# skim0119/gym-softrobot

Measured on AMD Instinct MI355X. Metric: env_steps_per_sec, higher is better.
Workload: dtype f64

## Files before the change

### gym_softrobot_amd/csrc/softrod_capi.hip

```cpp
#include <hip/hip_runtime.h>
#include <hip/hip_ext.h>

#include <cmath>
#include <cstdio>
#include <cstdlib>
#include <cstring>
#include <new>
#include <string>
#include <vector>

#include "softrod_kernels.hpp"
#include "softrod_dynamics_readout.hpp"
#include "softrod_copy_envs.hpp"
#include "softrod_state_bank.hpp"
#include "softrod_episode_stats.hpp"
#include "softrod_shape.hpp"
#include "softrod_reset_shapes.hpp"

using namespace softrod;

template <class Row>
struct EnvTable {
    Row* dev = nullptr;
    Row* host = nullptr;
// ... 39 lines not shown
    bool window_paired = true;
    std::string tier;
    RodParams P{};
    StatePtrs S{};
    std::vector<void*> owned;
    double* d_init = nullptr;
    uint8_t* d_mask = nullptr;
    double* d_basis = nullptr;
    double* d_spline = nullptr;
    bool spline_set = false;
    RodParams* d_params = nullptr;
    StatePtrs* d_state = nullptr;
    double* d_time_tab = nullptr;
    double* d_mat = nullptr;
    double* d_render_radius = nullptr;
    double* d_mtab = nullptr;
    bool muscles_set = false;
    unsigned* d_ticket = nullptr;
    bool tapered = false;
    bool was_reset = false;
    bool basis_set = false;
    double* h_init = nullptr;
    uint8_t* h_mask = nullptr;
    std::vector<hipEvent_t> ev_start, ev_stop;
    int timed = 0;
    hipEvent_t ev_reset = nullptr;
    int q_depth = 0;
    double* d_queue = nullptr;
    double* h_queue = nullptr;
    int* d_consumed = nullptr;
    int* d_produced = nullptr;
    int* d_underflow = nullptr;
    uint8_t* d_flags = nullptr;
    int* h_produced = nullptr;
    std::vector<int> seen_consumed;
    std::vector<int2> pending;
    double* h_stage = nullptr;
    int2* h_where = nullptr;
    double* d_stage = nullptr;
    int2* d_where = nullptr;
    size_t stage_cap = 0;
    int* h_status = nullptr;
    hipEvent_t ev_status = nullptr;
    bool status_pending = false;
    hipEvent_t ev_queue = nullptr;
    bool same_step = false;
// ... 275 lines not shown
    }
    SR_HIP(h, hipGetLastError());
    return SOFTROD_OK;
}

enum : unsigned { kOptMuscles = SOFTROD_FEAT_COOMM_MUSCLES, kOptEarlyTerm = kFeatEarlyTerm, kOptEnvMaterial = kFeatEnvMaterial,
                  kOptEnvContact = kFeatEnvContact, kOptCompiledFor = kOptEarlyTerm | kOptEnvMaterial | kOptEnvContact };
constexpr int kAny = -1, kMoctoEnvs = -2;
constexpr unsigned kAnyFeatures = kRuntimeFeatures;
using StepKernel = void (*)(RodParams, StatePtrs, const float*, float*, double*, uint8_t*, uint8_t*, double*, int, int, int);
using OctoKernel = void (*)(RodParams, StatePtrs, const float*, float*, double*, uint8_t*, uint8_t*, int, int, int);
using WindowKernel = void (*)(RodParams, StatePtrs, const float*, int, int);

struct StepRow {
    unsigned feats;
    int env;
    int math, epl;
    int taper, zup;
    int nw_min, nw_max;
    bool windowed;
    unsigned needs, honours;
    StepKernel step; OctoKernel octo; WindowKernel window;
    bool cert;
    int epb, waves;
    const char* label;
};

constexpr StepRow compiled_row(unsigned F, int env, int epl, int taper, int nw_min, int nw_max, const char* label) {
    const bool rt = F == kRuntimeFeatures;
    StepRow r{};
    r.feats = rt ? kAnyFeatures : F & ~(kFeatPlaneZup | kOptCompiledFor);
    r.env = env; r.math = SOFTROD_MATH_FAST; r.epl = epl; r.taper = taper; r.nw_min = nw_min; r.nw_max = nw_max;
    r.zup = rt ? kAny : (F & kFeatPlaneZup) != 0;
    r.needs = rt ? 0u : F & kOptCompiledFor;
    r.honours = rt ? 0u : F & (kOptCompiledFor | kOptMuscles);
    r.epb = 1; r.label = label;
    return r;
}
template <unsigned F, int E, int EPL, bool TAPER = false>
constexpr StepRow fast_row(const char* label) {
    StepRow r = compiled_row(F, E, EPL, TAPER, 1, 1, label);
    r.step = softrod_step_fast_kernel<F, E, EPL, TAPER>;
    r.cert = (F & ~kFeatEnvMaterial) == SOFTROD_FEATURES_SOFTPENDULUM;
    return r;
}
template <unsigned F, int MAXW, int EPB>
constexpr StepRow octo_row(int env, int nw_min, int nw_max, const char* label) {
    StepRow r = compiled_row(F, env, 1, kAny, nw_min, nw_max, label);
    r.octo = softrod_octo_step_kernel<F, MAXW, EPB>;
    r.epb = EPB; r.waves = EPB == 1 ? 0 : MAXW * EPB;
    return r;
}
template <unsigned F, int RPB>
constexpr StepRow window_row(const char* label) {
    StepRow r = compiled_row(F, SOFTROD_ENV_ARM_SINGLE, 2, 0, 1, 1, label);
    r.window = softrod_step_window_kernel<F, RPB>;
    r.windowed = true; r.epb = RPB; r.waves = 2 * RPB;
    return r;
}
template <bool ET>
constexpr StepRow libm_row(unsigned feats, int env, int zup, int taper, unsigned honours) {
    StepRow r{};
    r.feats = feats; r.env = env; r.math = SOFTROD_MATH_LIBM; r.epl = 1; r.taper = taper; r.zup = zup;
    r.nw_min = r.nw_max = r.epb = 1;
    r.needs = ET ? kOptEarlyTerm : 0u; r.honours = r.needs | kOptMuscles | honours;
    r.step = softrod_step_libm_kernel<ET>;
// ... 144 lines not shown
        SR_HIP(h, hipMalloc((void**)&T.dev, N * sizeof(Row)));
        SR_HIP(h, hipHostMalloc((void**)&T.host, N * sizeof(Row), hipHostMallocDefault));
        SR_HIP(h, hipEventCreateWithFlags(&T.ev, hipEventDisableTiming));
        Row R0;
        build(own, R0);
        for (size_t i = 0; i < N; ++i) T.host[i] = R0;
        if (const hipError_t e = bank_adopt_table(h, T.dev, R0)) {
            T.release();
            T = EnvTable<Row>{};
            return fail(h, SOFTROD_EHIP, std::string("state bank: ") + hipGetErrorString(e));
        }
        slot = T.dev;
        SR_HIP(h, hipMemcpy(h->d_state, &h->S, sizeof(StatePtrs), hipMemcpyHostToDevice));
    } else {
        SR_HIP(h, hipEventSynchronize(T.ev));
    }
    for (size_t i = 0; i < N; ++i)
        if (!mask || mask[i]) build(values + W * i, T.host[i]);
    SR_HIP(h, hipMemcpyAsync(T.dev, T.host, N * sizeof(Row), hipMemcpyHostToDevice, st));
    SR_HIP(h, hipEventRecord(T.ev, st));
    return SOFTROD_OK;
}

template <class K, class... A>
void launch_stamped(K kernel, const dim3& grid, const dim3& block, hipStream_t st, hipEvent_t t0, hipEvent_t t1, A... args) {
    if (t0 || t1) hipExtLaunchKernelGGL(kernel, grid, block, 0, st, t0, t1, 0, args...);
    else hipLaunchKernelGGL(kernel, grid, block, 0, st, args...);
}

int launch_step(softrod_handle* h, const float* actions, float* obs, double* reward,
                uint8_t* term, uint8_t* trunc, double* aux, int n_sub, int epilogue, int pack,
                hipStream_t st) {
    if (h->q_depth > 0 && epilogue && !h->same_step) {
        if (const int rc = launch_autoreset(h, obs, reward, term, trunc, aux, pack, st)) return rc;
        if (h->rs_count > 0)
            if (const int rc = launch_reset_shapes(h, kPickSkipped, nullptr, obs, term, trunc, aux, pack, st)) return rc;
    }
    if ((h->cfg.features & SOFTROD_FEAT_COOMM_MUSCLES) && h->cfg.math_mode == SOFTROD_MATH_FAST) {
        const bool push = h->cfg.env_kind == SOFTROD_ENV_ARM_PUSH || is_pull(h) || is_mocto(h);
        if (is_mocto(h) && (!h->tapered || !h->muscles_set || (h->cfg.env_kind == SOFTROD_ENV_ARM_TWO && !h->basis_set)))
            return fail(h, SOFTROD_EINVAL, "the muscle octopus needs softrod_set_radius_profile and softrod_set_muscle_layers "
                                           "(and SOFTROD_ENV_ARM_TWO softrod_set_action_basis) before it steps");
        if (push && !h->tapered)
            return fail(h, SOFTROD_EINVAL, "SOFTROD_ENV_ARM_PUSH (SOFTROD_MATH_FAST): call softrod_set_radius_profile first "
                                           "(the reference's arm is tapered, arm_push_env.py:160-179)");
        if (!push && h->tapered)
            return fail(h, SOFTROD_EINVAL, "a tapered muscle rod outside SOFTROD_ENV_ARM_PUSH runs under SOFTROD_MATH_LIBM only");
    }
    const StepChoice c = select_step(h, epilogue);
    if (!c.row) return fail(h, SOFTROD_EINVAL, c.why);
    const StepChoice after = c.row->windowed ? select_step(h, 0) : StepChoice{nullptr, nullptr};
    if (c.row->windowed && !after.row) return fail(h, SOFTROD_EINVAL, after.why);
    if (c.row->cert) h->cert_live = true;
    else if (const int rc = clear_planar_certs(h, st, false)) return rc;
    auto launch = [&](const StepRow& r, int n, int epi, hipEvent_t t0, hipEvent_t t1) {
        const dim3 grid((unsigned)((h->cfg.n_envs + r.epb - 1) / r.epb)), block(kLanes * (r.waves ? r.waves : h->nw));
        if (r.window) launch_stamped(r.window, grid, block, st, t0, t1, h->P, h->S, actions, n, h->window_refresh);
        else if (r.octo) launch_stamped(r.octo, grid, block, st, t0, t1, h->P, h->S, actions, obs, reward, term, trunc, n, epi, pack);
        else launch_stamped(r.step, grid, block, st, t0, t1, h->P, h->S, actions, obs, reward, term, trunc, aux, n, epi, pack);
    };
    const bool timing = h->timed < (int)h->ev_start.size();
    const hipEvent_t t0 = timing ? h->ev_start[h->timed] : nullptr, t1 = timing ? h->ev_stop[h->timed] : nullptr;
    const bool mocto = c.row->env == kMoctoEnvs;
    const bool action_first = mocto && epilogue && actions, epilogue_last = mocto && epilogue;
    const dim3 grid((unsigned)h->cfg.n_envs), block(kLanes * h->nw);
    if (action_first)
        launch_stamped(softrod_mocto_action_kernel, grid, block, st, t0, nullptr, h->P, h->S, actions, n_sub);
    launch(*c.row, n_sub, epilogue, action_first ? nullptr : t0, (after.row || epilogue_last) ? nullptr : t1);
    if (after.row) launch(*after.row, 0, 1, nullptr, epilogue_last ? nullptr : t1);
    if (epilogue_last)
        launch_stamped(softrod_mocto_epilogue_kernel, grid, block, st, nullptr, t1, h->P, h->S, obs, reward, term, trunc, 1, pack);
    SR_HIP(h, hipGetLastError());
    if (timing) ++h->timed;
    if (h->q_depth > 0 && epilogue && h->same_step) {
        if (const int rc = launch_autoreset_same_step(h, obs, aux, pack, st)) return rc;
        if (h->rs_count > 0)
            if (const int rc = launch_reset_shapes(h, kPickFinished, nullptr, obs, term, trunc, aux, pack, st)) return rc;
    }
    return SOFTROD_OK;
}

int upload_and_reset(softrod_handle* h, hipStream_t st, bool use_mask) {
    const size_t N = (size_t)h->cfg.n_envs;
    if (const int rc = clear_planar_certs(h, st)) return rc;
    SR_HIP(h, hipMemcpyAsync(h->d_init, h->h_init, N * h->init_stride * sizeof(double), hipMemcpyHostToDevice, st));
    if (use_mask)
        SR_HIP(h, hipMemcpyAsync(h->d_mask, h->h_mask, N, hipMemcpyHostToDevice, st));
    ResetArgs A{h->d_init, use_mask ? h->d_mask : nullptr};
    if (is_octo(h)) {
        OctoResetArgs OA{h->d_init, h->d_init + N * (size_t)h->cfg.n_arm * 18, use_mask ? h->d_mask : nullptr};
        hipLaunchKernelGGL(softrod_octo_reset_kernel, dim3((unsigned)N), dim3(kLanes * h->nw), 0, st, h->P, h->S, OA);
    } else
        hipLaunchKernelGGL(by_epl(h, softrod_reset_kernel<1>, softrod_reset_kernel<2>), dim3((unsigned)N), dim3(kLanes), 0, st,
                           h->P, h->S, A);
// ... 1848 lines not shown
    if (!h->S.planar_cert) return SOFTROD_OK;
    SR_ON_DEVICE(h);
    SR_HIP(h, hipDeviceSynchronize());
    std::vector<uint8_t> bytes((size_t)h->cfg.n_envs + 1, 0);
    bytes.back() = on ? 1 : 0;
    SR_HIP(h, hipMemcpy(h->S.planar_cert, bytes.data(), bytes.size(), hipMemcpyHostToDevice));
    h->cert_live = false;
    h->cert_on = on != 0;
    return SOFTROD_OK;
}

int softrod_planar_certificates(softrod_handle* h, uint8_t* out, void* stream) {
    if (!h || !out) return fail(h, SOFTROD_EINVAL, "planar certificates: null argument");
    SR_ON_DEVICE(h);
    const size_t N = (size_t)h->cfg.n_envs;
    if (!h->S.planar_cert) SR_HIP(h, hipMemsetAsync(out, 0, N, (hipStream_t)stream));
    else SR_HIP(h, hipMemcpyAsync(out, h->S.planar_cert, N, hipMemcpyDeviceToDevice, (hipStream_t)stream));
    return SOFTROD_OK;
}

int softrod_set_timing(softrod_handle* h, int n_launches) {
    if (!h || n_launches < 0 || n_launches > (1 << 20)) return fail(h, SOFTROD_EINVAL, "bad argument");
    SR_ON_DEVICE(h);
    while ((int)h->ev_start.size() < n_launches) {
        hipEvent_t a = nullptr, b = nullptr;
        SR_HIP(h, hipEventCreate(&a));
        SR_HIP(h, hipEventCreate(&b));
        h->ev_start.push_back(a);
        h->ev_stop.push_back(b);
    }
    while ((int)h->ev_start.size() > n_launches) {
        (void)hipEventDestroy(h->ev_start.back());
        (void)hipEventDestroy(h->ev_stop.back());
        h->ev_start.pop_back();
        h->ev_stop.pop_back();
    }
    h->timed = 0;
    return SOFTROD_OK;
}

int softrod_kernel_times_ms(softrod_handle* h, float* out_ms, int cap, int* count) {
    if (!h || !out_ms || !count || cap < 0) return fail(h, SOFTROD_EINVAL, "bad argument");
    SR_ON_DEVICE(h);
    const int n = h->timed < cap ? h->timed : cap;
    for (int i = 0; i < n; ++i) {
        SR_HIP(h, hipEventSynchronize(h->ev_stop[i]));
        SR_HIP(h, hipEventElapsedTime(out_ms + i, h->ev_start[i], h->ev_stop[i]));
    }
    *count = n;
    return SOFTROD_OK;
}

int softrod_last_kernel_ms(softrod_handle* h, float* ms) {
    if (!h || !ms) return fail(h, SOFTROD_EINVAL, "null argument");
    if (h->timed < 1) return fail(h, SOFTROD_EINVAL, "timing not enabled or no timed launch yet");
    SR_ON_DEVICE(h);
    SR_HIP(h, hipEventSynchronize(h->ev_stop[h->timed - 1]));
    SR_HIP(h, hipEventElapsedTime(ms, h->ev_start[h->timed - 1], h->ev_stop[h->timed - 1]));
    return SOFTROD_OK;
}

const char* softrod_last_error(softrod_handle* h) { return h ? h->err.c_str() : g_err.c_str(); }

const char* softrod_kernel_tier(softrod_handle* h) {
    if (!h) return "";
    const StepChoice c = select_step(h);
    std::string t = c.row ? c.row->label : std::string("none: ") + c.why;
    auto fill = [&t](const char* token, const std::string& with) {
        const size_t at = t.find(token);
        if (at != std::string::npos) t.replace(at, std::strlen(token), with);
    };
    fill("{waves}", std::to_string(h->nw) + (h->nw == 1 ? " wave" : " waves"));
    fill("{refresh}", std::to_string(h->window_refresh));
    if (c.row && c.row->windowed)
        if (const StepRow* after = select_step(h, 0).row) t += std::string(" + ") + after->label + " epilogue";
    if (h->env_mat.dev) t += ",env material";
    if (h->env_contact.dev) t += ",env contact";
    h->tier = t;
    return h->tier.c_str();
}

int softrod_destroy(softrod_handle* h) {
    if (!h) return SOFTROD_OK;
    DeviceGuard guard_(h->device);
    (void)hipDeviceSynchronize();
    autoreset_release(h);
    for (void* p : h->owned) (void)hipFree(p);
    for (double* p : h->d_rs_field) if (p) (void)hipFree(p);
    if (h->h_init) (void)hipHostFree(h->h_init);
    h->env_mat.release();
    h->env_contact.release();
    if (h->h_mask) (void)hipHostFree(h->h_mask);
    for (hipEvent_t e : h->ev_start) (void)hipEventDestroy(e);
    for (hipEvent_t e : h->ev_stop) (void)hipEventDestroy(e);
    if (h->ev_reset) (void)hipEventDestroy(h->ev_reset);
    if (h->h_pairs) (void)hipHostFree(h->h_pairs);
    if (h->ev_pairs) (void)hipEventDestroy(h->ev_pairs);
    h->bank.release();
    if (h->d_stats) (void)hipFree(h->d_stats);
    delete h;
    return SOFTROD_OK;
}

}

#ifdef SOFTROD_PHASE_CLOCKS
extern "C" int softrod_debug_phase_clocks(unsigned long long* out, int n_rods) {
    return (int)hipMemcpyFromSymbol(out, HIP_SYMBOL(softrod::g_phase_clock), (size_t)n_rods * 8 * sizeof(unsigned long long));
}
#endif
```

### gym_softrobot_amd/csrc/softrod_fast.hpp

```cpp
#pragma once

namespace softrod {

__device__ __forceinline__ bool wave_any(bool p) { return __builtin_amdgcn_ballot_w64(p) != 0ull; }
__device__ __forceinline__ bool wave_any_of(unsigned long long lanes, bool p) {
    return (__builtin_amdgcn_ballot_w64(p) & lanes) != 0ull;
}

__device__ __forceinline__ double horner(double g, double y, double c) {
    double d;
    asm("v_fma_f64 %0, %1, %2, %3" : "=v"(d) : "v"(g), "v"(y), "v"(c));
    return d;
}
__device__ __forceinline__ void fma_over(double& d, double a, double b, double c) {
    asm("v_fma_f64 %0, %1, %2, %3" : "+v"(d) : "v"(a), "v"(b), "v"(c));
}
__device__ __forceinline__ void fma_inplace_u(double& x, double m, double a) {
    asm("v_fma_f64 %0, %1, %0, %2" : "+v"(x) : "s"(m), "v"(a));
}

template <bool LEAN = true, bool ON_CIRCLE = false>
__device__ __forceinline__ void sinc_cosc(double t, double& sc, double& cc) {
    if (!wave_any(t >= 1.0e-3)) {
        if constexpr (LEAN) {
// ... 542 lines not shown
constexpr int fast_kernel_waves() {
    if (EPL > 1) return 1;
    if (F == kRuntimeFeatures) return SOFTROD_RUNTIME_WAVES;
    if (F & (SOFTROD_FEAT_PLANE_CONTACT_ANISO | SOFTROD_FEAT_LAPLACE_FILTER | SOFTROD_FEAT_SPLINE_MUSCLE_TORQUES |
             SOFTROD_FEAT_COOMM_MUSCLES))
        return SOFTROD_CONTACT_WAVES;
    if (TAPER) return SOFTROD_CONTACT_WAVES;
    return (F & ~kFeatEnvMaterial) == SOFTROD_FEATURES_SOFTPENDULUM ? SOFTROD_PLANAR_WAVES : SOFTROD_FAST_WAVES;
}

template <unsigned F, int E, int EPL, bool TAPER = false>
__global__ void __launch_bounds__(kLanes, (fast_kernel_waves<F, EPL, TAPER>()))
softrod_step_fast_kernel(const RodParams P, const StatePtrs S, const float* __restrict__ actions,
                         float* __restrict__ obs, double* __restrict__ reward,
                         uint8_t* __restrict__ terminated, uint8_t* __restrict__ truncated,
                         double* __restrict__ aux, const int n_sub, const int epilogue, const int pack) {
    const int rod = blockIdx.x;
    const int lane = threadIdx.x;
    const size_t N = (size_t)P.n_envs;
    [[maybe_unused]] EnvMaterial M;
    if constexpr (kEnvMaterial<F>) M = S.env_mat[rod];
    [[maybe_unused]] EnvContact CT;
    if constexpr (kEnvContact<F>) CT = S.env_contact[rod];
    if (epilogue && S.skip && S.skip[rod]) {
        if (lane == 0) S.skip[rod] = 0;
        if (lane == 0 && early_term_on<F>(P)) S.aux[rod] = 0.0;
        return;
    }

    __builtin_amdgcn_s_setprio(3);
    SR_PHASE(0);
    constexpr bool kPlanarKernel = (F & ~kFeatEnvMaterial) == SOFTROD_FEATURES_SOFTPENDULUM;
    LaneN<EPL> L;
    BcTargets B;
    EnvAction A;
    [[maybe_unused]] bool certified = false, cert_on = false, proof_ok = true, proof_nan = false;
    [[maybe_unused]] double s2w = 1.0;
    bool blown_up = false;
    if constexpr (kPlanarKernel) {
        unsigned cert = 0, on = 0;
        if (S.planar_cert) { on = S.planar_cert[N]; cert = S.planar_cert[rod]; }
        double bc_in_plane[3];
        planar_load_state<EPL>(S, N, rod, lane, L, bc_in_plane);
        set_action_n<F, E, EPL>(P, S, N, rod, lane, actions, A, B, L);
        cert_on = __builtin_amdgcn_readfirstlane((int)on) != 0;
        cert = cert_on ? (unsigned)__builtin_amdgcn_readfirstlane((int)cert) : 0u;
// ... 24 lines not shown
    if constexpr (kEnvMaterial<F>) build_const_m<F, EPL, TAPER>(P, M, lane, A, C, S.mat);
    else build_const_m<F, EPL, TAPER>(P, P, lane, A, C, S.mat);
    if constexpr (kEnvContact<F>) C.ct = CT;
    if constexpr (kMusclesCompiled<F>) build_muscle_const<F, EPL, true>(P, S, N, rod, lane, A, C);
    RodParams Pk = P;
    if (!has<F>(P, SOFTROD_FEAT_ANALYTICAL_DAMPER)) Pk.damp_t = 1.0;

    if constexpr (kPlanarKernel) {
        blown_up = n_sub > 0 && epilogue && __any(proof_nan || planar_has_nan<EPL>(P, lane, L));
    } else if (n_sub > 0 && epilogue && rod_has_nan<EPL>(P, lane, L)) {
        blown_up = true;
        poison_rod<EPL>(L);
        time = clock_after(P, S, time, n_sub);
    }
    if constexpr (kPlanarKernel) {
        PlanarN<EPL> Z;
        const bool planar = n_sub > 0 && !blown_up && !__any(!(planar_from_lane<EPL>(P, lane, L, s2w, Z) && proof_ok));
        if (__builtin_expect(planar, 1)) {
            PlanarC<EPL> K;
            planar_build_const<EPL, kEnvMaterial<F>>(Pk, C, lane, K);
            const double ta = P.time_two_half_adds ? P.half_dt : P.dt;
            const double tb = P.time_two_half_adds ? P.half_dt : 0.0;
            int tk = -1;
            if (S.time_tab && n_sub == P.tab_n_sub) {
                const double kf = rint(time * P.inv_step_time);
                const int k = (kf >= 0.0 && kf < (double)(P.tab_len - 1)) ? (int)kf : -1;
                tk = (k >= 0 && S.time_tab[k] == time) ? k : -1;
            }
            const double step_dt = EPL > 1 ? opaque_v(P.dt) : P.dt;
            SR_PHASE(2);
#if SOFTROD_PLANAR_EXEC_MASK
            if (lane * EPL <= P.n_elem) {
#endif
                planar_kinematic_n<EPL>(P.half_dt, K.hq_hdt, C, K, Z);
                {
                    int s = 0;
#pragma unroll
                    for (int q = 0; q < 4; ++q) {
                        if (q == 1) __builtin_amdgcn_s_setprio(2);
                        if (q == 2) __builtin_amdgcn_s_setprio(1);
                        if (q == 3) __builtin_amdgcn_s_setprio(0);
                        const int end = ProgressPriority::bound(n_sub - 1, q);
                        for (; s < end; ++s) {
                            planar_dynamic_n<EPL>(Pk, C, K, lane, Z);
#ifdef SOFTROD_DIAG_TWO_HALF_STEPS
                            planar_kinematic_n<EPL>(P.half_dt, K.hq_hdt, C, K, Z);
                            planar_kinematic_n<EPL>(P.half_dt, K.hq_hdt, C, K, Z);
#else
                            planar_kinematic_n<EPL>(step_dt, K.hq_dt, C, K, Z);
#endif
                        }
                    }
                }
                planar_dynamic_n<EPL>(Pk, C, K, lane, Z);
                planar_kinematic_n<EPL>(P.half_dt, K.hq_hdt, C, K, Z);
#if SOFTROD_PLANAR_EXEC_MASK
            }
#endif
            if (__builtin_amdgcn_readfirstlane(tk) >= 0) time = S.time_tab[tk + 1];
            else
                for (int s = 0; s < n_sub; ++s) time = (time + ta) + tb;
            SR_PHASE(3);
            planar_store<EPL>(S, N, rod, lane, Z, !SOFTROD_PLANAR_EXEC_MASK || lane * EPL <= P.n_elem, !certified);
            if (cert_on && !certified && lane == 0) S.planar_cert[rod] = Z.s2 > 0.0 ? 1 : 2;
#pragma unroll
            for (int s = 0; s < EPL; ++s) {
#pragma unroll
                for (int c = 0; c < 3; ++c) { L.x[s][c] = 0.0; L.v[s][c] = 0.0; L.w[s][c] = 0.0; L.t[s][c] = 0.0; }
#pragma unroll
                for (int c = 0; c < 9; ++c) L.Q[s][c] = 0.0;
            }
            planar_to_lane<EPL>(Z, L);
        } else {
            if (cert_on && lane == 0) S.planar_cert[rod] = 0;
            general_step_cold<F, E, EPL>(S.params, S.self, rod, lane, actions, n_sub, blown_up);
            __builtin_amdgcn_fence(__ATOMIC_ACQUIRE, "wavefront");
            load_lane<EPL, F>(S, N, rod, opaque_lane(lane), L);
            time = S.time[rod];
        }
    } else {
        if (n_sub > 0 && !blown_up) {
            general_substeps<F, EPL, TAPER>(P, Pk, C, B, lane, L, n_sub);
// ... 17 lines not shown
```

### gym_softrobot_amd/csrc/softrod_kernels.hpp

```cpp
#pragma once
#include <hip/hip_runtime.h>
#include <stdint.h>

#include "../../include/softrod.h"

namespace softrod {

constexpr int kLanes = 64;

constexpr unsigned kRuntimeFeatures = 0xFFFFFFFFu;
constexpr unsigned kFeaturesTaperedSuckerArm = SOFTROD_FEAT_ANALYTICAL_DAMPER | SOFTROD_FEAT_SUCKER_CONSTRAINT;
constexpr unsigned kFeatPlaneZup = 1u << 30;
constexpr unsigned kFeatEarlyTerm = 1u << 29;
constexpr unsigned kFeatEnvMaterial = 1u << 28;
template <unsigned F>
constexpr bool kEnvMaterial = F != kRuntimeFeatures && (F & kFeatEnvMaterial) != 0;
constexpr unsigned kFeatEnvContact = 1u << 27;
template <unsigned F>
constexpr bool kEnvContact = F != kRuntimeFeatures && (F & kFeatEnvContact) != 0;
constexpr int kRuntimeEnv = -1;
constexpr unsigned kFeaturesMuscleRod = SOFTROD_FEAT_FIXED_BC | SOFTROD_FEAT_ANALYTICAL_DAMPER | SOFTROD_FEAT_COOMM_MUSCLES;
template <unsigned F>
constexpr bool kMusclesCompiled = F != kRuntimeFeatures && (F & SOFTROD_FEAT_COOMM_MUSCLES) != 0;

struct RodParams {
// ... 73 lines not shown
    double* envmem;
    const double* basis;
    double* head;
    uint8_t* needs_reset;
    uint8_t* skip;
    const double* queue;
    int* q_consumed;
    const int* q_produced;
    int* q_underflow;
    int q_depth, q_record;
    const struct RodParams* params;
    const struct StatePtrs* self;
    const double* time_tab;
    const double* mat;
    double* sucker;
    int* sucker_idx;
    double* mact;
    const double* mtab;
    double* aux;
    float* prev_kappa;
    const EnvMaterial* env_mat;
    const EnvContact* env_contact;
    uint8_t* planar_cert;
};

__device__ __forceinline__ double from_next(double x) {
    int lo = __double2loint(x), hi = __double2hiint(x);
    lo = __builtin_amdgcn_mov_dpp(lo, 0x130, 0xf, 0xf, true);
    hi = __builtin_amdgcn_mov_dpp(hi, 0x130, 0xf, 0xf, true);
    return __hiloint2double(hi, lo);
}
__device__ __forceinline__ double from_prev(double x) {
    int lo = __double2loint(x), hi = __double2hiint(x);
    lo = __builtin_amdgcn_mov_dpp(lo, 0x138, 0xf, 0xf, true);
    hi = __builtin_amdgcn_mov_dpp(hi, 0x138, 0xf, 0xf, true);
    return __hiloint2double(hi, lo);
}

__device__ __forceinline__ double wave_sum(double x) {
#pragma unroll
    for (int off = 32; off >= 1; off >>= 1) x += __shfl_xor(x, off);
    return x;
}

template <unsigned F>
__device__ __forceinline__ bool has(const RodParams& P, unsigned bit) {
    if constexpr (F == kRuntimeFeatures) return (P.features & bit) != 0;
// ... 1468 lines not shown
    }
    if (P.features & SOFTROD_FEAT_ANALYTICAL_DAMPER) {
        L.v[0][0] *= M.damp_t; L.v[0][1] *= M.damp_t; L.v[0][2] *= M.damp_t;
        L.w[0][0] *= pow(M.damp_r[0], e);
        L.w[0][1] *= pow(M.damp_r[1], e);
        L.w[0][2] *= pow(M.damp_r[2], e);
    }
    if (P.features & SOFTROD_FEAT_LAPLACE_FILTER) laplace_filter_rates_n<1>(P, lane, L);
    if (P.damp_before_constrain) {
        constrain_rates_n<kRuntimeFeatures, 1>(P, B, lane, L);
        sucker_rates_n<kRuntimeFeatures, 1>(P, B, lane, L);
    }
}

#ifndef SOFTROD_LIBM_WAVES
#define SOFTROD_LIBM_WAVES 1
#endif
template <bool ET>
__global__ void __launch_bounds__(kLanes, SOFTROD_LIBM_WAVES)
softrod_step_libm_kernel(const RodParams P, const StatePtrs S, const float* __restrict__ actions,
                         float* __restrict__ obs, double* __restrict__ reward,
                         uint8_t* __restrict__ terminated, uint8_t* __restrict__ truncated,
                         double* __restrict__ aux, const int n_sub, const int epilogue, const int pack) {
    const int rod = blockIdx.x;
    const int lane = threadIdx.x;
    const size_t N = (size_t)P.n_envs;
    if (epilogue && S.skip && S.skip[rod]) {
        if (lane == 0) S.skip[rod] = 0;
        if (ET && lane == 0) S.aux[rod] = 0.0;
        return;
    }

    LaneN<1> L;
    load_lane<1, kRuntimeFeatures>(S, N, rod, lane, L);
    BcTargets B;
    load_bc(S, N, rod, B);
    load_suckers<kRuntimeFeatures>(P, S, N, rod, B);
    EnvAction A;
    set_action_n<kRuntimeFeatures, kRuntimeEnv, 1>(P, S, N, rod, lane, actions, A, B, L);
    if (epilogue) push_store_prev_com<kRuntimeFeatures, kRuntimeEnv, 1>(P, S, N, rod, lane, L, n_sub);
    ConstN<1> C;
    const EnvMaterial E = env_material_rt(P, S, rod);
    if (S.mat) build_const_m<kRuntimeFeatures, 1, true>(P, E, lane, A, C, S.mat);
    else build_const_m<kRuntimeFeatures, 1>(P, E, lane, A, C);
    build_muscle_const<kRuntimeFeatures, 1, false>(P, S, N, rod, lane, A, C);
    C.ct = env_contact_rt(P, S, rod);
// ... 224 lines not shown
```

### gym_softrobot_amd/csrc/softrod_mocto.hpp

```cpp
#pragma once

namespace softrod {

__device__ __forceinline__ bool is_mocto_env(int env) {
    return env == SOFTROD_ENV_CRAWL || env == SOFTROD_ENV_ARM_TWO || env == SOFTROD_ENV_REACH;
}

__device__ __forceinline__ int mocto_obs_dim(const RodParams& P) {
    const int n = P.n_elem, na = P.n_arm, nk = P.n_action;
    if (P.env_kind == SOFTROD_ENV_ARM_TWO) return na * ((n - 1) * 2 + nk + na + 3);
    return na * ((n - 1) + (n + 1) * 4 + nk + na + (P.env_kind == SOFTROD_ENV_CRAWL ? 17 : 18));
}

__device__ __forceinline__ float mocto_f32(double v) {
    const float f = (float)v;
    return isnan(f) ? 0.0f : (isinf(f) ? copysignf(3.4028234663852886e38f, f) : f);
}

__device__ __forceinline__ void mocto_write_obs(const RodParams& P, const StatePtrs& S, int env, int tid,
                                                const double x[3], const double v[3], double kap0,
                                                const HeadState& H, float* __restrict__ o) {
    const size_t N = (size_t)P.n_envs;
    const int n = P.n_elem, na = P.n_arm, nk = P.n_action;
    const int r = tid & (P.seg - 1), arm = tid >> P.seg_shift;
// ... 14 lines not shown
        return;
    }
    const int nt = P.env_kind == SOFTROD_ENV_CRAWL ? 2 : 3;
    const int width = (n - 1) + (n + 1) * 4 + nk + na + nt + 15;
    float* row = o + (size_t)arm * width;
    if (r < n - 1) row[r] = mocto_f32(kap0);
    if (r <= n) {
        row[(n - 1) + r] = mocto_f32(x[0]);
        row[(n - 1) + (n + 1) + r] = mocto_f32(x[1]);
        row[(n - 1) + 2 * (n + 1) + r] = mocto_f32(v[0]);
        row[(n - 1) + 3 * (n + 1) + r] = mocto_f32(v[1]);
    }
    const int off = (n - 1) + 4 * (n + 1);
    for (int q = r; q < nk; q += P.seg) row[off + q] = mocto_f32((double)pa[q]);
    for (int q = r; q < na; q += P.seg) row[off + nk + q] = (q == arm) ? 1.0f : 0.0f;
    float* sh = row + off + nk + na;
    if (r < nt) sh[r] = mocto_f32(S.aux[(size_t)r * N + env]);
    if (r < 3) { sh[nt + r] = mocto_f32(H.x[r]); sh[nt + 3 + r] = mocto_f32(H.v[r]); }
    if (r < 9) sh[nt + 6 + r] = mocto_f32(H.Q[r]);
}

__global__ void __launch_bounds__(1024)
softrod_mocto_action_kernel(const RodParams P, const StatePtrs S, const float* __restrict__ actions, const int n_sub) {
    const int env = blockIdx.x, tid = threadIdx.x;
    if (S.skip && S.skip[env]) return;
    const int lane = tid & 63, wave = tid >> 6, nw = blockDim.x >> 6;
    const size_t N = (size_t)P.n_envs, NR = N * (size_t)nw, NA = N * (size_t)P.n_arm;
    const size_t row = (size_t)env * nw + wave;
    const int n = P.n_elem, na = P.n_arm, nk = P.n_action;
    const int r = tid & (P.seg - 1), arm = tid >> P.seg_shift;
    const int adim = na * nk;
    const float* act = actions + (size_t)env * adim;
    if (arm < na) {
        const float* a = act + (size_t)arm * nk;
        const size_t ai = (size_t)env * na + arm;
        double* m0 = S.mact + ((size_t)0 * NR + row) * kLanes + lane;
        double* m1 = S.mact + ((size_t)1 * NR + row) * kLanes + lane;
        double* m2 = S.mact + ((size_t)2 * NR + row) * kLanes + lane;
        if (P.env_kind == SOFTROD_ENV_CRAWL) {
            if (r < n) *m2 = (double)a[1];
            if (r == 0) {
                const float loc = fminf(fmaxf(a[0] * (float)n, 0.0f), (float)(n - 1));
                S.sucker_idx[ai] = (int)loc;
                S.sucker[ai] = (double)a[2];
            }
        } else if (P.env_kind == SOFTROD_ENV_ARM_TWO) {
// ... 6 lines not shown
                    s0 = fma(b, fmax(lm, 0.0), s0);
                    s1 = fma(b, fabs(fmin(lm, 0.0)), s1);
                    s2 = fma(b, (double)a[6 + j], s2);
                }
                *m0 = s0; *m1 = s1; *m2 = s2;
            }
            if (r < 3) S.sucker[(size_t)r * NA + ai] = (double)a[r];
        } else {
            if (r < n) { *m0 = (double)a[r]; *m1 = (double)a[n + r]; *m2 = (double)a[2 * n + r]; }
        }
    }
    for (int q = tid; q < adim; q += blockDim.x) S.prev_action[(size_t)env * adim + q] = act[q];
    if (tid == 0 && n_sub > 0) {
        S.aux[(size_t)3 * N + env] = S.head[(size_t)0 * N + env];
        S.aux[(size_t)4 * N + env] = S.head[(size_t)1 * N + env];
    }
}

__global__ void __launch_bounds__(1024)
softrod_mocto_epilogue_kernel(const RodParams P, const StatePtrs S, float* __restrict__ obs,
                              double* __restrict__ reward, uint8_t* __restrict__ terminated,
                              uint8_t* __restrict__ truncated, const int scalars, const int pack) {
    __shared__ double tipd[16];
    const int env = blockIdx.x, tid = threadIdx.x;
    if (scalars && S.skip && S.skip[env]) {
        __syncthreads();
        if (tid == 0) S.skip[env] = 0;
        return;
    }
    const int lane = tid & 63, wave = tid >> 6, nw = blockDim.x >> 6;
    const size_t N = (size_t)P.n_envs, NR = N * (size_t)nw;
    const size_t m = ((size_t)env * nw + wave) * kLanes + lane;
    const int n = P.n_elem, na = P.n_arm;
    const int r = tid & (P.seg - 1), arm = tid >> P.seg_shift;
    double x[3], v[3];
#pragma unroll
    for (int c = 0; c < 3; ++c) { x[c] = S.pos[c * NR * kLanes + m]; v[c] = S.vel[c * NR * kLanes + m]; }
    const double kap0 = S.kap[m];
    HeadState H;
    double unused[2];
    load_head(S, N, env, H, unused);
    const int od = mocto_obs_dim(P);
    float* o = out_row(obs, env, od, pack);
    mocto_write_obs(P, S, env, tid, x, v, kap0, H, o);
    if (!scalars) return;
    const bool node = arm < na && r <= n;
// ... 51 lines not shown
```

### gym_softrobot_amd/csrc/softrod_octo.hpp

```cpp
#pragma once

namespace softrod {

struct HeadState {
    double x[3], v[3], Q[9], w[3];
};

__device__ __forceinline__ void load_head(const StatePtrs& S, size_t N, int env, HeadState& H, double tgt[2]) {
#pragma unroll
    for (int i = 0; i < 3; ++i) {
        H.x[i] = S.head[(size_t)i * N + env];
        H.v[i] = S.head[(size_t)(3 + i) * N + env];
        H.w[i] = S.head[(size_t)(15 + i) * N + env];
    }
#pragma unroll
    for (int i = 0; i < 9; ++i) H.Q[i] = S.head[(size_t)(6 + i) * N + env];
    tgt[0] = S.head[(size_t)18 * N + env];
    tgt[1] = S.head[(size_t)19 * N + env];
}

__device__ __forceinline__ void store_head(const StatePtrs& S, size_t N, int env, const HeadState& H) {
#pragma unroll
    for (int i = 0; i < 3; ++i) {
        S.head[(size_t)i * N + env] = H.x[i];
// ... 105 lines not shown

#ifndef SOFTROD_OCTO_WAVES
#define SOFTROD_OCTO_WAVES 2
#endif
#ifndef SOFTROD_MUSCLE_OCTO_WAVES
#define SOFTROD_MUSCLE_OCTO_WAVES 1
#endif
template <unsigned F>
constexpr int octo_kernel_waves() { return kMusclesCompiled<F> ? SOFTROD_MUSCLE_OCTO_WAVES : SOFTROD_OCTO_WAVES; }

template <unsigned F, int MAXW, int EPB = 1>
__global__ void __launch_bounds__(kLanes * MAXW * EPB, (octo_kernel_waves<F>()))
softrod_octo_step_kernel(const RodParams P, const StatePtrs S, const float* __restrict__ actions,
                         float* __restrict__ obs, double* __restrict__ reward,
                         uint8_t* __restrict__ terminated, uint8_t* __restrict__ truncated,
                         const int n_sub, const int epilogue, const int pack) {
    static_assert(EPB == 1 || MAXW == 2, "several envs per workgroup: the two-wave shape only");
    __shared__ double xch_[EPB][2][MAXW][4];
    __shared__ double sxy_[EPB][kLanes * MAXW][2];
    __shared__ int scount_[EPB];
    __shared__ int flag_[EPB][2][MAXW];
    __shared__ int sany_[2][EPB];

    const int wib = threadIdx.x >> 6;
    const int es = (EPB == 1) ? 0 : (wib & (EPB - 1));
    const int wave = (EPB == 1) ? wib : (wib / EPB);
    const int lane = threadIdx.x & 63;
    const int tid = wave * kLanes + lane;
    const int nw = (EPB == 1) ? (int)(blockDim.x >> 6) : MAXW;
    const int nthr = nw * kLanes;
    const bool active = (EPB == 1) || ((int)blockIdx.x * EPB + es < P.n_envs);
    const int env = active ? (int)blockIdx.x * EPB + es : P.n_envs - 1;
    auto& xch = xch_[es];
    auto& sxy = sxy_[es];
    int& scount = scount_[es];
    const size_t N = (size_t)P.n_envs, NR = N * (size_t)nw;
    const int row = env * nw + wave;
    const int n = P.n_elem, nk = P.n_action;
    const int r = tid & (P.seg - 1), arm = tid >> P.seg_shift;
    const bool arm_ok = arm < P.n_arm;
    if constexpr (kEnvContact<F>)
        stage_contact_params_env(P, tid == 0 ? S.env_contact + env : nullptr, es);
    else if constexpr ((F & kFeatPlaneZup) != 0) stage_contact_params(P);
    if (tid < 2 * MAXW * 4) (&xch[0][0][0])[tid] = 0.0;
    if constexpr (EPB == 1) __syncthreads();
    if (EPB > 1 && tid < 2 * MAXW) (&flag_[es][0][0])[tid] = 0;
// ... 451 lines not shown
```

### gym_softrobot_amd/csrc/softrod_planar.hpp

```cpp
#pragma once

namespace softrod {

template <int EPL>
struct PlanarN {
    double x[EPL][2], v[EPL][2];
    double c[EPL], s[EPL];
    double s2;
    double wz[EPL];
    double t[EPL][2];
    double dl[EPL];
    double d[EPL][2];
    double dv[EPL][2];
};

template <int EPL>
struct PlanarC {
    double cfy[EPL], cay[EPL];
    double cwl[EPL];
    double bk[EPL];
    double bke[EPL];
    double xl[EPL];
    double hq_dt[EPL], hq_hdt[EPL];
    double jr;
// ... 203 lines not shown

template <int EPL>
__device__ __forceinline__ void planar_to_lane(const PlanarN<EPL>& Z, LaneN<EPL>& L) {
#pragma unroll
    for (int s = 0; s < EPL; ++s) {
        L.x[s][0] = Z.x[s][0]; L.x[s][1] = Z.x[s][1];
        L.v[s][0] = Z.v[s][0]; L.v[s][1] = Z.v[s][1];
        L.Q[s][0] = -Z.s2 * Z.s[s]; L.Q[s][1] = Z.s2 * Z.c[s];
        L.Q[s][6] = Z.c[s]; L.Q[s][7] = Z.s[s];
        L.w[s][1] = Z.s2 * Z.wz[s];
        L.t[s][0] = Z.t[s][0]; L.t[s][1] = Z.t[s][1]; L.t[s][2] = 0.0;
    }
}

template <int EPL>
__device__ __forceinline__ void planar_store(const StatePtrs& S, size_t N, int rod, int lane, const PlanarN<EPL>& Z,
                                             bool stepped, bool tan_z) {
    constexpr size_t W = (size_t)kLanes * EPL;
    const size_t base = (size_t)rod * W + (size_t)opaque_lane(lane) * EPL;
    if (tan_z) {
#pragma unroll
        for (int s = 0; s < EPL; ++s) S.tan[2 * N * W + base + s] = 0.0;
    }
#pragma unroll
    for (int s = 0; s < EPL; ++s) {
        S.dir[0 * N * W + base + s] = -Z.s2 * Z.s[s];
        S.dir[1 * N * W + base + s] = Z.s2 * Z.c[s];
        S.omg[1 * N * W + base + s] = Z.s2 * Z.wz[s];
    }
    if (stepped) {
#pragma unroll
        for (int s = 0; s < EPL; ++s) {
#pragma unroll
            for (int c = 0; c < 2; ++c) {
                S.pos[c * N * W + base + s] = Z.x[s][c];
                S.vel[c * N * W + base + s] = Z.v[s][c];
                S.tan[c * N * W + base + s] = Z.t[s][c];
            }
            S.dir[6 * N * W + base + s] = Z.c[s];
            S.dir[7 * N * W + base + s] = Z.s[s];
        }
    }
}

template <int EPL>
__device__ __forceinline__ void planar_kinematic_n(double h, const double (&hq_h)[EPL], const ConstN<EPL>& C,
                                                   const PlanarC<EPL>& K, PlanarN<EPL>& Z) {
    double ra[EPL], ran[EPL];
#pragma unroll
    for (int s = 0; s < EPL; ++s) {
        const double hp = h * C.hx[s];
// ... 133 lines not shown
```

### gym_softrobot_amd/csrc/softrod_window.hpp

```cpp
#pragma once

namespace softrod {

constexpr int kWindowRho = 4;

template <unsigned F>
__device__ __forceinline__ void window_load(const StatePtrs& S, size_t N, int rod, int g, LaneN<1>& L) {
    constexpr size_t W = 2 * kLanes;
    const size_t m = (size_t)rod * W + (size_t)g;
#pragma unroll
    for (int c = 0; c < 3; ++c) {
        L.x[0][c] = S.pos[c * N * W + m];
        L.v[0][c] = S.vel[c * N * W + m];
        L.w[0][c] = S.omg[c * N * W + m];
        L.t[0][c] = S.tan[c * N * W + m];
        L.kap[0][c] = S.kap[c * N * W + m];
        L.rk[0][c] = S.rkap[c * N * W + m];
    }
#pragma unroll
    for (int c = 0; c < 9; ++c) L.Q[0][c] = S.dir[c * N * W + m];
}

__device__ __forceinline__ void window_store(const StatePtrs& S, size_t N, int rod, int g, const LaneN<1>& L) {
    constexpr size_t W = 2 * kLanes;
// ... 2 lines not shown
    for (int c = 0; c < 3; ++c) {
        S.pos[c * N * W + m] = L.x[0][c];
        S.vel[c * N * W + m] = L.v[0][c];
        S.omg[c * N * W + m] = L.w[0][c];
        S.tan[c * N * W + m] = L.t[0][c];
        S.kap[c * N * W + m] = L.kap[0][c];
    }
#pragma unroll
    for (int c = 0; c < 9; ++c) S.dir[c * N * W + m] = L.Q[0][c];
}

template <unsigned F, int RPB = 1>
__global__ void __launch_bounds__(2 * kLanes * RPB, SOFTROD_CONTACT_WAVES)
softrod_step_window_kernel(const RodParams P, const StatePtrs S, const float* __restrict__ actions,
                           const int n_sub, const int refresh) {
    static_assert(RPB == 1 || RPB == 4, "one rod per workgroup, or four with partner waves on one SIMD");
    constexpr int kFields = 18;
    constexpr int kHalo = (RPB == 1) ? kLanes : 32;
    constexpr int kBuf = (RPB == 1) ? 1 : 2;
    __shared__ double ex_[RPB][kBuf][2][kFields][kHalo];
    __shared__ int flag_[RPB][2];
    __shared__ int sany_[RPB];

    const int wib = threadIdx.x >> 6;
    const int es = (RPB == 1) ? 0 : (wib & (RPB - 1));
    const int wave = (RPB == 1) ? wib : (wib / RPB);
    const int lane = threadIdx.x & 63;
    const int tid = wave * kLanes + lane;
    const bool active = (RPB == 1) || ((int)blockIdx.x * RPB + es < P.n_envs);
    const int rod = active ? (int)blockIdx.x * RPB + es : P.n_envs - 1;
    auto& ex = ex_[es];
    const size_t N = (size_t)P.n_envs;
    const int n = P.n_elem;
    bool live = active && !(S.skip && S.skip[rod]);
    if constexpr (RPB == 1) { if (!live) return; }
    const int off = wave ? (n + 1 - kLanes) : 0;
    const int g = off + lane;
    const int split = (n + 1) / 2;
    const bool owned = wave ? (g >= split) : (g < split);
    const int gi = (wave == 0 && lane == kLanes - 1) ? n : g;
    if constexpr (RPB > 1) {
        if (tid < 2) flag_[es][tid] = 0;
        if (tid == 0) sany_[es] = 0;
    }

    LaneN<1> L;
// ... 112 lines not shown
```

Baseline: 14.50 million.

## Replace per-launch event timing with in-kernel wall-clock stamps; trim planar stores

Most kernels now record per-wave wall-clock entry and exit times into a device ring through relaxed atomics, instead of being launched with hipExtLaunchKernelGGL start and stop events. Events are now created lazily and kept only for fast-kernel variants that do not stamp themselves. The fast step also loads the next time-table entry up front and broadcasts it with readfirstlane, and the planar writeback skips dir/omg stores when a rod neither stepped nor has tan_z set. Event-stamped launches add per-launch overhead when timing is on; the in-kernel stamps add a few atomics per wave and a shared-memory slot.

Result: no change. 14.60 million, median of 2 (+0.8%).

```diff
diff --git a/gym_softrobot_amd/csrc/softrod_capi.hip b/gym_softrobot_amd/csrc/softrod_capi.hip
--- a/gym_softrobot_amd/csrc/softrod_capi.hip
+++ b/gym_softrobot_amd/csrc/softrod_capi.hip
@@ -85,6 +85,8 @@
     bool basis_set = false;
     double* h_init = nullptr;
     uint8_t* h_mask = nullptr;
+    unsigned long long* d_stamps = nullptr;
+    int ring_len = 0, ring_cap = 0;
     std::vector<hipEvent_t> ev_start, ev_stop;
     int timed = 0;
     hipEvent_t ev_reset = nullptr;
@@ -406,6 +408,7 @@
     unsigned needs, honours;
     StepKernel step; OctoKernel octo; WindowKernel window;
     bool cert;
+    bool by_events;
     int epb, waves;
     const char* label;
 };
@@ -426,6 +429,7 @@
     StepRow r = compiled_row(F, E, EPL, TAPER, 1, 1, label);
     r.step = softrod_step_fast_kernel<F, E, EPL, TAPER>;
     r.cert = (F & ~kFeatEnvMaterial) == SOFTROD_FEATURES_SOFTPENDULUM;
+    r.by_events = !kStampsItself<F>;
     return r;
 }
 template <unsigned F, int MAXW, int EPB>
@@ -616,11 +620,7 @@
     return SOFTROD_OK;
 }
 
-template <class K, class... A>
-void launch_stamped(K kernel, const dim3& grid, const dim3& block, hipStream_t st, hipEvent_t t0, hipEvent_t t1, A... args) {
-    if (t0 || t1) hipExtLaunchKernelGGL(kernel, grid, block, 0, st, t0, t1, 0, args...);
-    else hipLaunchKernelGGL(kernel, grid, block, 0, st, args...);
-}
+constexpr size_t kStampEntry = (size_t)kStampShards * kStampWords;
 
 int launch_step(softrod_handle* h, const float* actions, float* obs, double* reward,
                 uint8_t* term, uint8_t* trunc, double* aux, int n_sub, int epilogue, int pack,
@@ -647,23 +647,31 @@
     if (c.row->windowed && !after.row) return fail(h, SOFTROD_EINVAL, after.why);
     if (c.row->cert) h->cert_live = true;
     else if (const int rc = clear_planar_certs(h, st, false)) return rc;
-    auto launch = [&](const StepRow& r, int n, int epi, hipEvent_t t0, hipEvent_t t1) {
+    const bool timing = h->timed < h->ring_len;
+    StatePtrs S = h->S;
+    S.stamp = timing ? h->d_stamps + (size_t)h->timed * kStampEntry : nullptr;
+    auto launch = [&](const StepRow& r, int n, int epi) {
         const dim3 grid((unsigned)((h->cfg.n_envs + r.epb - 1) / r.epb)), block(kLanes * (r.waves ? r.waves : h->nw));
-        if (r.window) launch_stamped(r.window, grid, block, st, t0, t1, h->P, h->S, actions, n, h->window_refresh);
-        else if (r.octo) launch_stamped(r.octo, grid, block, st, t0, t1, h->P, h->S, actions, obs, reward, term, trunc, n, epi, pack);
-        else launch_stamped(r.step, grid, block, st, t0, t1, h->P, h->S, actions, obs, reward, term, trunc, aux, n, epi, pack);
+        if (r.window) hipLaunchKernelGGL(r.window, grid, block, 0, st, h->P, S, actions, n, h->window_refresh);
+        else if (r.octo) hipLaunchKernelGGL(r.octo, grid, block, 0, st, h->P, S, actions, obs, reward, term, trunc, n, epi, pack);
+        else if (timing && r.by_events) {
+            h->ev_start.resize((size_t)h->ring_len, nullptr);
+            h->ev_stop.resize((size_t)h->ring_len, nullptr);
+            hipEvent_t& t0 = h->ev_start[h->timed];
+            hipEvent_t& t1 = h->ev_stop[h->timed];
+            if (!t0 && (hipEventCreate(&t0) != hipSuccess || hipEventCreate(&t1) != hipSuccess)) return;
+            hipExtLaunchKernelGGL(r.step, grid, block, 0, st, t0, t1, 0, h->P, S, actions, obs, reward, term, trunc, aux, n, epi, pack);
+        } else hipLaunchKernelGGL(r.step, grid, block, 0, st, h->P, S, actions, obs, reward, term, trunc, aux, n, epi, pack);
     };
-    const bool timing = h->timed < (int)h->ev_start.size();
-    const hipEvent_t t0 = timing ? h->ev_start[h->timed] : nullptr, t1 = timing ? h->ev_stop[h->timed] : nullptr;
     const bool mocto = c.row->env == kMoctoEnvs;
     const bool action_first = mocto && epilogue && actions, epilogue_last = mocto && epilogue;
     const dim3 grid((unsigned)h->cfg.n_envs), block(kLanes * h->nw);
     if (action_first)
-        launch_stamped(softrod_mocto_action_kernel, grid, block, st, t0, nullptr, h->P, h->S, actions, n_sub);
-    launch(*c.row, n_sub, epilogue, action_first ? nullptr : t0, (after.row || epilogue_last) ? nullptr : t1);
-    if (after.row) launch(*after.row, 0, 1, nullptr, epilogue_last ? nullptr : t1);
+        hipLaunchKernelGGL(softrod_mocto_action_kernel, grid, block, 0, st, h->P, S, actions, n_sub);
+    launch(*c.row, n_sub, epilogue);
+    if (after.row) launch(*after.row, 0, 1);
     if (epilogue_last)
-        launch_stamped(softrod_mocto_epilogue_kernel, grid, block, st, nullptr, t1, h->P, h->S, obs, reward, term, trunc, 1, pack);
+        hipLaunchKernelGGL(softrod_mocto_epilogue_kernel, grid, block, 0, st, h->P, S, obs, reward, term, trunc, 1, pack);
     SR_HIP(h, hipGetLastError());
     if (timing) ++h->timed;
     if (h->q_depth > 0 && epilogue && h->same_step) {
@@ -2558,20 +2566,50 @@
 int softrod_set_timing(softrod_handle* h, int n_launches) {
     if (!h || n_launches < 0 || n_launches > (1 << 20)) return fail(h, SOFTROD_EINVAL, "bad argument");
     SR_ON_DEVICE(h);
-    while ((int)h->ev_start.size() < n_launches) {
-        hipEvent_t a = nullptr, b = nullptr;
-        SR_HIP(h, hipEventCreate(&a));
-        SR_HIP(h, hipEventCreate(&b));
-        h->ev_start.push_back(a);
-        h->ev_stop.push_back(b);
-    }
-    while ((int)h->ev_start.size() > n_launches) {
-        (void)hipEventDestroy(h->ev_start.back());
-        (void)hipEventDestroy(h->ev_stop.back());
-        h->ev_start.pop_back();
-        h->ev_stop.pop_back();
-    }
+    if (n_launches > h->ring_cap) {
+        if (h->d_stamps) SR_HIP(h, hipFree(h->d_stamps));
+        h->d_stamps = nullptr;
+        h->ring_cap = h->ring_len = 0;
+        SR_HIP(h, hipMalloc(&h->d_stamps, (size_t)n_launches * kStampEntry * sizeof(unsigned long long)));
+        h->ring_cap = n_launches;
+    }
+    if (n_launches > 0) {
+        std::vector<unsigned long long> clear((size_t)n_launches * kStampEntry, 0ull);
+        for (size_t i = 0; i < clear.size(); i += kStampWords) clear[i] = ~0ull;
+        SR_HIP(h, hipMemcpy(h->d_stamps, clear.data(), clear.size() * sizeof(unsigned long long), hipMemcpyHostToDevice));
+    }
+    for (hipEvent_t e : h->ev_start) if (e) (void)hipEventDestroy(e);
+    for (hipEvent_t e : h->ev_stop) if (e) (void)hipEventDestroy(e);
+    h->ev_start.clear();
+    h->ev_stop.clear();
+    h->ring_len = n_launches;
     h->timed = 0;
+    return SOFTROD_OK;
+}
+
+static int read_stamps(softrod_handle* h, int first, int n, float* out_ms) {
+    if (n < 1) return SOFTROD_OK;
+    int khz = 0;
+    SR_HIP(h, hipDeviceGetAttribute(&khz, hipDeviceAttributeWallClockRate, h->device));
+    if (khz <= 0) return fail(h, SOFTROD_EHIP, "the device reports no wall clock rate");
+    std::vector<unsigned long long> ring((size_t)n * kStampEntry);
+    SR_HIP(h, hipDeviceSynchronize());
+    SR_HIP(h, hipMemcpy(ring.data(), h->d_stamps + (size_t)first * kStampEntry, ring.size() * sizeof(unsigned long long),
+                        hipMemcpyDeviceToHost));
+    for (int i = 0; i < n; ++i) {
+        const size_t e = (size_t)(first + i);
+        if (e < h->ev_start.size() && h->ev_start[e]) {
+            SR_HIP(h, hipEventElapsedTime(out_ms + i, h->ev_start[e], h->ev_stop[e]));
+            continue;
+        }
+        unsigned long long t_in = ~0ull, t_out = 0ull;
+        for (size_t l = 0; l < (size_t)kStampShards; ++l) {
+            const unsigned long long* line = ring.data() + (size_t)i * kStampEntry + l * kStampWords;
+            if (line[0] < t_in) t_in = line[0];
+            if (line[1] > t_out) t_out = line[1];
+        }
+        out_ms[i] = t_out > t_in ? (float)((double)(t_out - t_in) / (double)khz) : 0.0f;
+    }
     return SOFTROD_OK;
 }
 
@@ -2579,10 +2617,7 @@
     if (!h || !out_ms || !count || cap < 0) return fail(h, SOFTROD_EINVAL, "bad argument");
     SR_ON_DEVICE(h);
     const int n = h->timed < cap ? h->timed : cap;
-    for (int i = 0; i < n; ++i) {
-        SR_HIP(h, hipEventSynchronize(h->ev_stop[i]));
-        SR_HIP(h, hipEventElapsedTime(out_ms + i, h->ev_start[i], h->ev_stop[i]));
-    }
+    if (const int rc = read_stamps(h, 0, n, out_ms)) return rc;
     *count = n;
     return SOFTROD_OK;
 }
@@ -2591,9 +2626,7 @@
     if (!h || !ms) return fail(h, SOFTROD_EINVAL, "null argument");
     if (h->timed < 1) return fail(h, SOFTROD_EINVAL, "timing not enabled or no timed launch yet");
     SR_ON_DEVICE(h);
-    SR_HIP(h, hipEventSynchronize(h->ev_stop[h->timed - 1]));
-    SR_HIP(h, hipEventElapsedTime(ms, h->ev_start[h->timed - 1], h->ev_stop[h->timed - 1]));
-    return SOFTROD_OK;
+    return read_stamps(h, h->timed - 1, 1, ms);
 }
 
 const char* softrod_last_error(softrod_handle* h) { return h ? h->err.c_str() : g_err.c_str(); }
@@ -2627,8 +2660,9 @@
     h->env_mat.release();
     h->env_contact.release();
     if (h->h_mask) (void)hipHostFree(h->h_mask);
-    for (hipEvent_t e : h->ev_start) (void)hipEventDestroy(e);
-    for (hipEvent_t e : h->ev_stop) (void)hipEventDestroy(e);
+    if (h->d_stamps) (void)hipFree(h->d_stamps);
+    for (hipEvent_t e : h->ev_start) if (e) (void)hipEventDestroy(e);
+    for (hipEvent_t e : h->ev_stop) if (e) (void)hipEventDestroy(e);
     if (h->ev_reset) (void)hipEventDestroy(h->ev_reset);
     if (h->h_pairs) (void)hipHostFree(h->h_pairs);
     if (h->ev_pairs) (void)hipEventDestroy(h->ev_pairs);
diff --git a/gym_softrobot_amd/csrc/softrod_fast.hpp b/gym_softrobot_amd/csrc/softrod_fast.hpp
--- a/gym_softrobot_amd/csrc/softrod_fast.hpp
+++ b/gym_softrobot_amd/csrc/softrod_fast.hpp
@@ -588,6 +588,7 @@
     if constexpr (kEnvMaterial<F>) M = S.env_mat[rod];
     [[maybe_unused]] EnvContact CT;
     if constexpr (kEnvContact<F>) CT = S.env_contact[rod];
+    [[maybe_unused]] const std::conditional_t<kStampsItself<F>, WaveStamp, NoStamp> stamp(S);
     if (epilogue && S.skip && S.skip[rod]) {
         if (lane == 0) S.skip[rod] = 0;
         if (lane == 0 && early_term_on<F>(P)) S.aux[rod] = 0.0;
@@ -658,11 +659,19 @@
             const double ta = P.time_two_half_adds ? P.half_dt : P.dt;
             const double tb = P.time_two_half_adds ? P.half_dt : 0.0;
             int tk = -1;
+            double t_next = time;
             if (S.time_tab && n_sub == P.tab_n_sub) {
                 const double kf = rint(time * P.inv_step_time);
                 const int k = (kf >= 0.0 && kf < (double)(P.tab_len - 1)) ? (int)kf : -1;
-                tk = (k >= 0 && S.time_tab[k] == time) ? k : -1;
+                if (k >= 0) {
+                    const double t_k = S.time_tab[k];
+                    t_next = S.time_tab[k + 1];
+                    tk = t_k == time ? k : -1;
+                }
             }
+            tk = __builtin_amdgcn_readfirstlane(tk);
+            t_next = __hiloint2double(__builtin_amdgcn_readfirstlane(__double2hiint(t_next)),
+                                      __builtin_amdgcn_readfirstlane(__double2loint(t_next)));
             const double step_dt = EPL > 1 ? opaque_v(P.dt) : P.dt;
             SR_PHASE(2);
 #if SOFTROD_PLANAR_EXEC_MASK
@@ -693,7 +702,7 @@
 #if SOFTROD_PLANAR_EXEC_MASK
             }
 #endif
-            if (__builtin_amdgcn_readfirstlane(tk) >= 0) time = S.time_tab[tk + 1];
+            if (tk >= 0) time = t_next;
             else
                 for (int s = 0; s < n_sub; ++s) time = (time + ta) + tb;
             SR_PHASE(3);
diff --git a/gym_softrobot_amd/csrc/softrod_kernels.hpp b/gym_softrobot_amd/csrc/softrod_kernels.hpp
--- a/gym_softrobot_amd/csrc/softrod_kernels.hpp
+++ b/gym_softrobot_amd/csrc/softrod_kernels.hpp
@@ -1,6 +1,7 @@
 #pragma once
 #include <hip/hip_runtime.h>
 #include <stdint.h>
+#include <type_traits>
 
 #include "../../include/softrod.h"
 
@@ -120,7 +121,31 @@
     const EnvMaterial* env_mat;
     const EnvContact* env_contact;
     uint8_t* planar_cert;
+    unsigned long long* stamp;
 };
+
+constexpr int kStampShards = 32, kStampWords = 8;
+struct WaveStamp {
+    const StatePtrs& S;
+    __device__ __forceinline__ static unsigned long long* entry_clock() {
+        __shared__ unsigned long long t_in[1024 / kLanes];
+        return t_in + threadIdx.x / kLanes;
+    }
+    __device__ __forceinline__ explicit WaveStamp(const StatePtrs& S_) : S(S_) {
+        if (S.stamp && (threadIdx.x & (kLanes - 1)) == 0) *entry_clock() = wall_clock64();
+    }
+    WaveStamp(const WaveStamp&) = delete;
+    __device__ __forceinline__ ~WaveStamp() {
+        if (S.stamp && (threadIdx.x & (kLanes - 1)) == 0) {
+            unsigned long long* line = S.stamp + ((blockIdx.x + threadIdx.x / kLanes) & (kStampShards - 1)) * kStampWords;
+            __hip_atomic_fetch_min(line, *entry_clock(), __ATOMIC_RELAXED, __HIP_MEMORY_SCOPE_AGENT);
+            __hip_atomic_fetch_max(line + 1, (unsigned long long)wall_clock64(), __ATOMIC_RELAXED, __HIP_MEMORY_SCOPE_AGENT);
+        }
+    }
+};
+struct NoStamp { __device__ __forceinline__ explicit NoStamp(const StatePtrs&) {} };
+template <unsigned F>
+constexpr bool kStampsItself = !(kEnvMaterial<F> && kEnvContact<F>);
 
 __device__ __forceinline__ double from_next(double x) {
     int lo = __double2loint(x), hi = __double2hiint(x);
@@ -1635,6 +1660,7 @@
                          float* __restrict__ obs, double* __restrict__ reward,
                          uint8_t* __restrict__ terminated, uint8_t* __restrict__ truncated,
                          double* __restrict__ aux, const int n_sub, const int epilogue, const int pack) {
+    const WaveStamp stamp(S);
     const int rod = blockIdx.x;
     const int lane = threadIdx.x;
     const size_t N = (size_t)P.n_envs;
diff --git a/gym_softrobot_amd/csrc/softrod_mocto.hpp b/gym_softrobot_amd/csrc/softrod_mocto.hpp
--- a/gym_softrobot_amd/csrc/softrod_mocto.hpp
+++ b/gym_softrobot_amd/csrc/softrod_mocto.hpp
@@ -60,6 +60,7 @@
 
 __global__ void __launch_bounds__(1024)
 softrod_mocto_action_kernel(const RodParams P, const StatePtrs S, const float* __restrict__ actions, const int n_sub) {
+    const WaveStamp stamp(S);
     const int env = blockIdx.x, tid = threadIdx.x;
     if (S.skip && S.skip[env]) return;
     const int lane = tid & 63, wave = tid >> 6, nw = blockDim.x >> 6;
@@ -112,6 +113,7 @@
                               double* __restrict__ reward, uint8_t* __restrict__ terminated,
                               uint8_t* __restrict__ truncated, const int scalars, const int pack) {
     __shared__ double tipd[16];
+    const WaveStamp stamp(S);
     const int env = blockIdx.x, tid = threadIdx.x;
     if (scalars && S.skip && S.skip[env]) {
         __syncthreads();
diff --git a/gym_softrobot_amd/csrc/softrod_octo.hpp b/gym_softrobot_amd/csrc/softrod_octo.hpp
--- a/gym_softrobot_amd/csrc/softrod_octo.hpp
+++ b/gym_softrobot_amd/csrc/softrod_octo.hpp
@@ -151,6 +151,7 @@
     __shared__ int flag_[EPB][2][MAXW];
     __shared__ int sany_[2][EPB];
 
+    const WaveStamp stamp(S);
     const int wib = threadIdx.x >> 6;
     const int es = (EPB == 1) ? 0 : (wib & (EPB - 1));
     const int wave = (EPB == 1) ? wib : (wib / EPB);
diff --git a/gym_softrobot_amd/csrc/softrod_planar.hpp b/gym_softrobot_amd/csrc/softrod_planar.hpp
--- a/gym_softrobot_amd/csrc/softrod_planar.hpp
+++ b/gym_softrobot_amd/csrc/softrod_planar.hpp
@@ -249,11 +249,13 @@
 #pragma unroll
         for (int s = 0; s < EPL; ++s) S.tan[2 * N * W + base + s] = 0.0;
     }
-#pragma unroll
-    for (int s = 0; s < EPL; ++s) {
-        S.dir[0 * N * W + base + s] = -Z.s2 * Z.s[s];
-        S.dir[1 * N * W + base + s] = Z.s2 * Z.c[s];
-        S.omg[1 * N * W + base + s] = Z.s2 * Z.wz[s];
+    if (stepped || tan_z) {
+#pragma unroll
+        for (int s = 0; s < EPL; ++s) {
+            S.dir[0 * N * W + base + s] = -Z.s2 * Z.s[s];
+            S.dir[1 * N * W + base + s] = Z.s2 * Z.c[s];
+            S.omg[1 * N * W + base + s] = Z.s2 * Z.wz[s];
+        }
     }
     if (stepped) {
 #pragma unroll
diff --git a/gym_softrobot_amd/csrc/softrod_window.hpp b/gym_softrobot_amd/csrc/softrod_window.hpp
--- a/gym_softrobot_amd/csrc/softrod_window.hpp
+++ b/gym_softrobot_amd/csrc/softrod_window.hpp
@@ -48,6 +48,7 @@
     __shared__ int flag_[RPB][2];
     __shared__ int sany_[RPB];
 
+    const WaveStamp stamp(S);
     const int wib = threadIdx.x >> 6;
     const int es = (RPB == 1) ? 0 : (wib & (RPB - 1));
     const int wave = (RPB == 1) ? wib : (wib / RPB);
```
